# alipay/PainlessInferenceAcceleration

Hardware: NVIDIA H100
Metric: accepted tokens/sec @ Llama-2-7B 64-draft/8-branch; mean accepted len/step (higher is better)
Workload: dtype bf16

## Files before the change

include/pia_b200.h:

```cpp
#ifndef PIA_B200_H_
#define PIA_B200_H_

#include <stdint.h>

#ifdef __cplusplus
extern "C" {
#endif

#define PIA_ABI_VERSION 2

typedef enum {
  PIA_OK = 0,
  PIA_ERR_INVALID = -1,
  PIA_ERR_INDEX = -2,
  PIA_ERR_CAPACITY = -3,
  PIA_ERR_CUDA = -4,
  PIA_ERR_UNSUPPORTED = -5
} pia_status;

const char *pia_last_error(void);
int pia_abi_version(void);
unsigned long long pia_launch_count(void);

typedef struct pia_trie pia_trie_t;
// ... 70 lines not shown
  const int32_t *d_pad_len;
  int64_t kv_slot_stride;
  int32_t kv_first_slot;
} pia_slots_t;

typedef struct pia_attn_plan pia_attn_plan_t;

typedef struct {
  int32_t n_q_heads, n_kv_heads, head_dim;
  int32_t max_seq;
  int32_t max_nodes;
  int32_t n_layers;
  int32_t kv_split_max;
  int32_t n_slots;
} pia_attn_config_t;

int pia_attn_plan_create(const pia_attn_config_t *cfg, void *d_k_cache, void *d_v_cache, pia_attn_plan_t **out);
int pia_attn_plan_destroy(pia_attn_plan_t *p);
int pia_attn_plan_set_debug(pia_attn_plan_t *p, void *d_timestamps);
int pia_attn_plan_grid(const pia_attn_plan_t *p, int *n_split, int *n_groups);

int pia_tree_attn_fwd(pia_attn_plan_t *p, int layer, const void *d_q, const uint64_t *d_mask, const pia_slots_t *slots,
                      float scale_mul, void *d_out, void *stream);

int pia_tree_attn_fused_fwd(pia_attn_plan_t *p, int layer, const void *d_qkv, const void *d_cos, const void *d_sin,
                            int max_pos, const uint64_t *d_mask, const pia_slots_t *slots, float scale_mul, void *d_out,
                            void *stream);

typedef struct pia_gemm_plan pia_gemm_plan_t;
int pia_gemm_plan_create(const void *d_w, int N, int K, const void *d_x, int x_rows, int split_k, int w_tiled,
                         pia_gemm_plan_t **out);
int pia_gemm_plan_create_grouped(const void *d_w, int groups, int N, int K, const void *d_x, int x_rows,
                                 pia_gemm_plan_t **out);
int pia_gemm_plan_destroy(pia_gemm_plan_t *g);
int pia_gemm_plan_splits(const pia_gemm_plan_t *g);
int pia_gemm_plan_set_pdl(pia_gemm_plan_t *g, int on);
int pia_gemm_plan_set_silu(pia_gemm_plan_t *g, int on);
int pia_gemm_run(pia_gemm_plan_t *g, int rows, void *d_out, void *stream);

int pia_rmsnorm(const void *d_x, const void *d_residual_in, const void *d_weight, float eps, int rows, int hidden,
                void *d_residual_out, void *d_y, void *stream);
int pia_rmsnorm_partials(const float *d_x_parts, int n_parts, int64_t part_stride, const void *d_residual_in,
                         const void *d_weight, float eps, int rows, int hidden, void *d_residual_out, void *d_y,
                         void *stream);
int pia_rope_kv_append(const void *d_qkv, const uint64_t *d_mask, int mask_words, const pia_slots_t *slots,
                       int n_q_heads, int n_kv_heads, int head_dim, const void *d_cos, const void *d_sin, int max_pos,
// ... 47 lines not shown
```

painlessinferenceacceleration_b200/_lib.py:

```python
import ctypes as C
import os

from .build import SO

_lib = None

i32p = C.POINTER(C.c_int32)
u64p = C.POINTER(C.c_uint64)
vp = C.c_void_p

PIA_OK, PIA_ERR_INVALID, PIA_ERR_INDEX, PIA_ERR_CAPACITY, PIA_ERR_CUDA, PIA_ERR_UNSUPPORTED = 0, -1, -2, -3, -4, -5
MODE = {'input': 0, 'output': 1, 'mix': 2}
GET_HIER, GET_ONE = 0, 1
GET_TAIL = 1
GET_FIRST_ONLY = 2


class TrieConfig(C.Structure):
    _fields_ = [('vocab_capacity', C.c_int32), ('node_capacity', C.c_int64), ('edge_capacity', C.c_int64),
                ('n_input_slots', C.c_int32), ('max_node', C.c_int32), ('max_output_node', C.c_int32),
                ('max_put_tokens', C.c_int32), ('frontier_capacity', C.c_int32), ('max_resident_queries', C.c_int32)]


class TrieStats(C.Structure):
# ... 28 lines not shown
    'pia_trie_set_limits': (C.c_int, [vp, C.c_int, C.c_int]),
    'pia_trie_put': (C.c_int, [vp, vp, C.c_int, vp, C.c_int, C.c_int, C.c_int, C.c_int, vp]),
    'pia_trie_tree_put': (C.c_int, [vp, C.c_int, vp, C.c_int, C.c_int, C.c_int, vp]),
    'pia_trie_stream_put': (C.c_int, [vp, vp, C.c_int, vp, C.c_int, C.c_int, vp, C.c_int, vp]),
    'pia_trie_get': (C.c_int, [vp, vp, vp, C.c_int, C.c_int, C.c_int, vp, C.c_int, C.c_int, C.c_int, C.c_int, C.c_int,
                               C.c_int, C.c_int, C.c_int, C.c_int, vp, vp, vp, vp, vp, vp, vp, vp]),
    'pia_trie_tree_squeeze': (C.c_int, [vp, C.c_int, vp]),
    'pia_trie_tree_reset_input_freq': (C.c_int, [vp, C.c_int, C.c_int, vp]),
    'pia_trie_reset_input_freqs': (C.c_int, [vp, C.c_int, vp]),
    'pia_trie_squeeze_branch_counts': (C.c_int, [vp, vp]),
    'pia_trie_fresh': (C.c_int, [vp, vp]),
    'pia_trie_stats': (C.c_int, [vp, C.POINTER(TrieStats), vp]),
    'pia_trie_copy_error_flags': (C.c_int, [vp, vp, vp]),
    'pia_trie_tree_counters': (C.c_int, [vp, C.c_int, C.POINTER(C.c_int64), C.POINTER(C.c_int64), vp]),
    'pia_trie_compact': (C.c_int, [vp, C.POINTER(C.c_int64), C.POINTER(C.c_int64), vp]),
    'pia_trie_export_sizes': (C.c_int, [vp, C.POINTER(C.c_int64), C.POINTER(C.c_int64), vp]),
    'pia_trie_export': (C.c_int, [vp, vp, C.c_int64, vp, C.c_int64, vp, vp, vp, vp]),
    'pia_trie_import': (C.c_int, [vp, vp, C.c_int64, vp, C.c_int64, vp, vp, vp, vp]),
    'pia_attn_plan_create': (C.c_int, [C.POINTER(AttnConfig), vp, vp, C.POINTER(vp)]),
    'pia_attn_plan_destroy': (C.c_int, [vp]),
    'pia_attn_plan_set_debug': (C.c_int, [vp, vp]),
    'pia_attn_plan_grid': (C.c_int, [vp, C.POINTER(C.c_int), C.POINTER(C.c_int)]),
    'pia_tree_attn_fwd': (C.c_int, [vp, C.c_int, vp, vp, C.POINTER(Slots), C.c_float, vp, vp]),
    'pia_tree_attn_fused_fwd': (C.c_int, [vp, C.c_int, vp, vp, vp, C.c_int, vp, C.POINTER(Slots), C.c_float, vp, vp]),
    'pia_rmsnorm': (C.c_int, [vp, vp, vp, C.c_float, C.c_int, C.c_int, vp, vp, vp]),
    'pia_rmsnorm_partials': (C.c_int, [vp, C.c_int, C.c_int64, vp, vp, C.c_float, C.c_int, C.c_int, vp, vp, vp]),
    'pia_gemm_plan_create': (C.c_int, [vp, C.c_int, C.c_int, vp, C.c_int, C.c_int, C.c_int, C.POINTER(vp)]),
    'pia_gemm_plan_create_grouped': (C.c_int, [vp, C.c_int, C.c_int, C.c_int, vp, C.c_int, C.POINTER(vp)]),
    'pia_gemm_plan_destroy': (C.c_int, [vp]),
    'pia_gemm_plan_splits': (C.c_int, [vp]),
    'pia_gemm_plan_set_pdl': (C.c_int, [vp, C.c_int]),
    'pia_gemm_plan_set_silu': (C.c_int, [vp, C.c_int]),
    'pia_gemm_run': (C.c_int, [vp, C.c_int, vp, vp]),
    'pia_rope_kv_append': (C.c_int, [vp, vp, C.c_int, C.POINTER(Slots), C.c_int, C.c_int, C.c_int, vp, vp,
                                     C.c_int, vp, vp, vp, C.c_int, vp]),
    'pia_silu_mul': (C.c_int, [vp, C.c_int, C.c_int, vp, vp]),
    'pia_embed_gather': (C.c_int, [vp, vp, vp, C.c_int, C.c_int, vp, vp]),
    'pia_moe_combine': (C.c_int, [vp, vp, C.c_int, C.c_int, C.c_int, C.c_int, vp, vp]),
    'pia_moe_router': (C.c_int, [vp, vp, C.c_int, C.c_int, C.c_int, C.c_int, vp, vp]),
    'pia_l2_prefetch': (C.c_int, [vp, C.c_int64, C.c_int64, C.c_int64, C.c_float, vp]),
    'pia_accept': (C.c_int, [C.POINTER(AcceptConfig), vp, vp, vp, C.c_int, C.c_int, C.c_int, vp, vp, vp, C.c_int, vp,
                             vp, vp, vp, vp, vp, vp, vp, vp]),
    'pia_accept_workspace_bytes': (C.c_int64, [C.POINTER(AcceptConfig)]),
    'pia_kv_compact': (C.c_int, [vp, vp, C.c_int, C.c_int, C.c_int, C.c_int, C.c_int, C.c_int64, vp, C.c_int, vp, vp,
                                 vp]),
    'pia_flood_update_draft_table': (C.c_int, [vp, C.c_int, vp, vp, C.c_int64, C.c_int, C.c_int, C.c_int, vp]),
# ... 36 lines not shown
```

painlessinferenceacceleration_b200/common/ops.py:

```python
import ctypes as C

import torch

from .. import _lib as L


def _s():
    return torch.cuda.current_stream().cuda_stream


def _p(t):
    return t.data_ptr() if t is not None else None


def rmsnorm(x, residual_in, weight, eps, residual_out, y):
    rows, hidden = x.shape
    L.check(L.load().pia_rmsnorm(_p(x), _p(residual_in), _p(weight), float(eps), rows, hidden, _p(residual_out),
                                 _p(y), _s()))


def rmsnorm_partials(parts, residual_in, weight, eps, residual_out, y):
    n_parts, prow, hidden = parts.shape
    rows = y.shape[0]
    L.check(L.load().pia_rmsnorm_partials(_p(parts), n_parts, prow * hidden, _p(residual_in), _p(weight), float(eps),
# ... 124 lines not shown
    L.check(L.load().pia_l2_prefetch(t.data_ptr() + offset_bytes, int(n_ranges), int(stride_bytes), int(range_bytes),
                                     float(gbytes_per_s), _s()))


def embed_gather(table, ids, n, out):
    rows, hidden = out.shape
    L.check(L.load().pia_embed_gather(_p(table), _p(ids), _p(n), rows, hidden, _p(out), _s()))


class AttnPlan(object):

    def __init__(self, k_cache, v_cache, n_q_heads, n_kv_heads, head_dim, max_nodes, kv_split_max=0):
        n_slots = k_cache.shape[0] if k_cache.dim() == 5 else 1
        n_layers, hkv, max_seq, hd = k_cache.shape[-4:]
        assert hkv == n_kv_heads and hd == head_dim and k_cache.is_contiguous() and v_cache.is_contiguous()
        self.cfg = L.AttnConfig(n_q_heads, n_kv_heads, head_dim, max_seq, max_nodes, n_layers, kv_split_max, n_slots)
        self.slot_stride = n_layers * hkv * max_seq * hd
        self.h = L.vp()
        self.lib = L.load()
        with torch.cuda.device(k_cache.device):
            L.check(self.lib.pia_attn_plan_create(C.byref(self.cfg), _p(k_cache), _p(v_cache), C.byref(self.h)))
        self._keep = (k_cache, v_cache)

    def forward(self, layer, q, mask, slots, out, scale_mul=1.0):
        assert q.shape[0] >= slots.rows and mask.shape[0] >= slots.rows and out.shape[0] >= slots.rows
        L.check(self.lib.pia_tree_attn_fwd(self.h, layer, _p(q), _p(mask), slots.ref(), float(scale_mul), _p(out), _s()))

    def forward_fused(self, layer, qkv, mask, slots, cos, sin, out, scale_mul=1.0):
        assert qkv.shape[0] >= slots.rows and mask.shape[0] >= slots.rows and out.shape[0] >= slots.rows
        L.check(self.lib.pia_tree_attn_fused_fwd(self.h, layer, _p(qkv), _p(cos), _p(sin), cos.shape[0], _p(mask),
                                                 slots.ref(), float(scale_mul), _p(out), _s()))

    def close(self):
        if self.h:
            self.lib.pia_attn_plan_destroy(self.h)
            self.h = None

    def __del__(self):
        try:
            self.close()
        except Exception:
            pass


class Accept(object):

    def __init__(self, vocab, max_nodes, repetition_penalty, eos_ids, max_length, device, bound_walk=False):
        eos = [int(e) for e in (eos_ids or []) if e is not None][:8]
        arr = (C.c_int32 * 8)(*(eos + [-1] * (8 - len(eos))))
# ... 27 lines not shown
```

painlessinferenceacceleration_b200/csrc/tree_attn.cu:

```cuda
#include <cuda.h>
#include <cuda_bf16.h>

#include <stdlib.h>

#include <new>

#include "common.cuh"

namespace pia {
namespace attn {

constexpr int BN = 128;
constexpr int HD = 128;
constexpr int NSTAGE = 2;
constexpr int NTHREADS = 288;
constexpr int PRODUCER_WARP = 8;
constexpr int SUB = 128 * 128;
constexpr int TILE_BYTES = 2 * SUB;
constexpr int SMEM_Q = 0, SMEM_K = TILE_BYTES, SMEM_V = SMEM_K + NSTAGE * TILE_BYTES;
constexpr int SMEM_BAR = SMEM_V + NSTAGE * TILE_BYTES;
constexpr int MRG_ACC = 0;
constexpr int MRG_ML = 112 * 1024;
constexpr int MRG_DED_ACC = SMEM_BAR + 256, MRG_DED_ACC_BYTES = (64 + 8) * 128 * 4,
               MRG_DED_ML = MRG_DED_ACC + MRG_DED_ACC_BYTES;
constexpr int SMEM_TOTAL = MRG_DED_ML + 1024 + 1024;
constexpr int MAX_SPLIT = 8;
// ... 93 lines not shown
  for (int j = 0; j < 8; ++j) {
    const float x = __bfloat162float(a.h[j]);
    const float r = lower ? -__bfloat162float(b.h[j]) : __bfloat162float(b.h[j]);
    o.h[j] = __float2bfloat16_rn(bfr(x * __bfloat162float(c.h[j])) + bfr(r * __bfloat162float(s.h[j])));
  }
  return o.u;
}

struct Params {
  const __nv_bfloat16 *q;
  const unsigned long long *mask;
  pia_slots_t sl;
  int slot_planes;
  int plane0;
  int layer, n_q_heads, n_kv_heads, np, mask_words, heads_per_cta, max_seq, n_split, tiles_per_cta;
  float scale_log2;
  int fused;
  const __nv_bfloat16 *qkv;
  const __nv_bfloat16 *cos_t, *sin_t;
  int max_pos;
  __nv_bfloat16 *kc_layer, *vc_layer;
  __nv_bfloat16 *out;
  unsigned long long *dbg;
};

__device__ __forceinline__ unsigned long long gtime() {
  unsigned long long t;
  asm volatile("mov.u64 %0, %%globaltimer;" : "=l"(t));
  return t;
}
#define DBG(ev) do { if (p.dbg) p.dbg[((size_t)blockIdx.y * gridDim.x + blockIdx.x) * 16 + (ev)] = gtime(); } while (0)

__global__ void __launch_bounds__(NTHREADS, 1)
k_tree_attn(const __grid_constant__ CUtensorMap map_k, const __grid_constant__ CUtensorMap map_v, Params p) {
  extern __shared__ uint8_t smem_raw[];
  const uint32_t base = (smem_u32(smem_raw) + 1023u) & ~1023u;
  uint8_t *sm = smem_raw + (base - smem_u32(smem_raw));
  const int tid = threadIdx.x, warp = tid >> 5, lane = tid & 31;

  const uint32_t bar0 = base + SMEM_BAR;
  const uint32_t bar_kv_full = bar0, bar_kv_empty = bar0 + 8 * NSTAGE, bar_v_full = bar0 + 16 * NSTAGE;

  pdl_launch_dependents();
  if (tid == 0) {
    asm volatile("prefetch.tensormap [%0];" ::"l"(reinterpret_cast<unsigned long long>(&map_k)) : "memory");
    asm volatile("prefetch.tensormap [%0];" ::"l"(reinterpret_cast<unsigned long long>(&map_v)) : "memory");
  }
  const int split = blockIdx.x, group = blockIdx.y;
  const int slot = blockIdx.z;
  const int n = p.sl.d_n[slot], P = p.sl.d_prefix_len[slot];
  const int pad_len = p.sl.d_pad_len ? p.sl.d_pad_len[slot] : 0;
  if (n <= 0) return;
  const long long row0 = (long long)slot * p.sl.rows_per_slot;
  const int L = P + n;
  const int hq0 = group * p.heads_per_cta;
  const int hkv = hq0 / (p.n_q_heads / p.n_kv_heads);
  const bool fused = p.fused != 0;
  const int Tp = (P + BN - 1) / BN;
  const int tiles_total = fused ? Tp + 1 : (L + BN - 1) / BN;
  const int rows_used = p.heads_per_cta * p.np;
  const int n_wg = rows_used / 64;
  const bool ded = (rows_used + MAX_SPLIT) * HD * 4 <= MRG_DED_ACC_BYTES;
  int ns = (tiles_total + p.tiles_per_cta - 1) / p.tiles_per_cta;
  if (ns > p.n_split) ns = p.n_split;
  if (ns < 1) ns = 1;
  if (split >= ns) {
    if (ns > 1) { cluster_sync_all(); cluster_sync_all(); }
    return;
  }
  const int tps = (tiles_total + ns - 1) / ns;
  const int t0 = split * tps;
  int t1 = t0 + tps;
  if (t1 > tiles_total) t1 = tiles_total;
  const int ntile = t1 - t0;
  const bool has_draft = fused && ntile > 0 && t1 == tiles_total;
  auto tile_of = [&](int i) -> int { return has_draft ? (i == 0 ? Tp : t0 + i - 1) : t0 + i; };
  if (ns > 1 && ded) cluster_arrive();
  auto barrier_a = [&]() { if (ded) cluster_wait(); else cluster_sync_all(); };
  const int mrg_acc = ded ? MRG_DED_ACC : MRG_ACC, mrg_ml = ded ? MRG_DED_ML : MRG_ML;
  const int mrg_stride = ded ? 64 + MAX_SPLIT : 128 + MAX_SPLIT;
  if (tid == 0) DBG(0);

  if (tid == 0) {
    for (int s = 0; s < NSTAGE; ++s) {
      mbar_init(bar_kv_full + 8 * s, 1); mbar_init(bar_v_full + 8 * s, 1);
      mbar_init(bar_kv_empty + 8 * s, 4 * n_wg);
    }
    asm volatile("fence.mbarrier_init.release.cluster;" ::: "memory");
  }
  __syncwarp();
  __syncthreads();
  if (tid == 0) DBG(1);

  if (warp == PRODUCER_WARP) {
    if (lane == 0 && ntile > 0) {
      const int plane = p.plane0 + slot * p.slot_planes + p.layer * p.n_kv_heads + hkv;
      int p_safe = P;
      if (p.slot_planes == 0) for (int b2 = 0; b2 < p.sl.batch; ++b2) p_safe = min(p_safe, p.sl.d_prefix_len[b2]);
      bool waited = false;
      for (int i = 0; i < ntile; ++i) {
        const int s = i % NSTAGE, ph = (i / NSTAGE) & 1;
        if (has_draft && i == 0) {
          mbar_arrive(bar_kv_full);
          mbar_arrive(bar_v_full);
          continue;
        }
        const int key0 = tile_of(i) * BN;
        if (!fused && !waited && key0 + BN > p_safe) { pdl_wait(); waited = true; }
        mbar_wait(bar_kv_empty + 8 * s, ph ^ 1);
        const uint32_t kd = base + SMEM_K + s * TILE_BYTES, vd = base + SMEM_V + s * TILE_BYTES;
        mbar_expect_tx(bar_kv_full + 8 * s, TILE_BYTES);
        tma_load_3d(kd, &map_k, bar_kv_full + 8 * s, 0, key0, plane);
        tma_load_3d(kd + SUB, &map_k, bar_kv_full + 8 * s, 64, key0, plane);
        mbar_expect_tx(bar_v_full + 8 * s, TILE_BYTES);
        tma_load_3d(vd, &map_v, bar_v_full + 8 * s, 0, key0, plane);
        tma_load_3d(vd + SUB, &map_v, bar_v_full + 8 * s, 64, key0, plane);
        if (i == 0) DBG(2);
      }
    }
    __syncwarp();
    if (ns > 1) { barrier_a(); cluster_sync_all(); }
  } else {
    pdl_wait();
    {
      const int srow = tid & 127, half = tid >> 7;
      const int hs = srow / p.np, node = srow % p.np;
      if (srow < rows_used) {
        if (!fused) {
          uint4 qv[8];
          const bool have = hs < p.heads_per_cta && node < n;
          const uint4 *src = reinterpret_cast<const uint4 *>(p.q + ((row0 + node) * p.n_q_heads + hq0 + hs) * HD) + half * 8;
#pragma unroll
          for (int ch = 0; ch < 8; ++ch) qv[ch] = have ? src[ch] : make_uint4(0, 0, 0, 0);
#pragma unroll
          for (int ch = 0; ch < 8; ++ch)
            *reinterpret_cast<uint4 *>(sm + SMEM_Q + half * SUB + srow * 128 + ((ch ^ (srow & 7)) << 4)) = qv[ch];
        } else {
          unsigned long long mr0 = 0ull, mr1 = 0ull;
          if (node < n) {
            mr0 = p.mask[(row0 + node) * p.mask_words];
            if (p.mask_words > 1) mr1 = p.mask[(row0 + node) * p.mask_words + 1];
          }
          int pos = (P > pad_len ? P - pad_len : 0) + __popcll(mr0) + __popcll(mr1) - 1;
          pos = pos < 0 ? 0 : (pos >= p.max_pos ? p.max_pos - 1 : pos);
// ... 201 lines not shown
        __syncwarp();
        if (lane == 0) mbar_arrive(bar_kv_empty + 8 * s);
      }
      if (tid == 0) DBG(8);
#pragma unroll
      for (int h = 0; h < 2; ++h) {
        l_run[h] += __shfl_xor_sync(FULL, l_run[h], 1);
        l_run[h] += __shfl_xor_sync(FULL, l_run[h], 2);
      }
      if (tid == 0) DBG(9);
      if (ns == 1) {
#pragma unroll
        for (int h = 0; h < 2; ++h) {
          if (live[h]) {
            const float inv = l_run[h] > 0.f ? 1.f / l_run[h] : 0.f;
            uint32_t *dst = reinterpret_cast<uint32_t *>(p.out + ((row0 + node[h]) * p.n_q_heads + hq0 + hs[h]) * HD);
#pragma unroll
            for (int nb = 0; nb < 16; ++nb) {
              __nv_bfloat162 b = __floats2bfloat162_rn(o[4 * nb + 2 * h] * inv, o[4 * nb + 2 * h + 1] * inv);
              dst[4 * nb + (lane & 3)] = *reinterpret_cast<uint32_t *>(&b);
            }
          }
        }
      } else {
        barrier_a();
        if (tid == 0) DBG(14);
        const int RS = (rows_used + ns - 1) / ns;
#pragma unroll
        for (int h = 0; h < 2; ++h) {
          if (live[h]) {
            const int owner = rw[h] / RS, rl = rw[h] % RS;
            const uint32_t dst = map_to_cta(base + mrg_acc + (uint32_t)((((lane & 3) >> 1) * mrg_stride + split * RS + rl) * 16 + (lane & 1) * 8), owner);
#pragma unroll
            for (int nb = 0; nb < 16; ++nb)
              st_cluster_f2(dst + (uint32_t)(2 * nb * mrg_stride) * 16, o[4 * nb + 2 * h], o[4 * nb + 2 * h + 1]);
            if ((lane & 3) == 0) st_cluster_f2(map_to_cta(base + mrg_ml + (uint32_t)(split * RS + rl) * 8, owner), m_run[h], l_run[h]);
          }
        }
        __syncwarp();
        if (tid == 0) DBG(15);
        cluster_sync_all();
      }
      if (tid == 0) DBG(10);
    } else {
      if (ns > 1) { barrier_a(); cluster_sync_all(); }
    }
  }
  if (ns > 1) {
    const int RS = (rows_used + ns - 1) / ns;
    const float4 *macc = reinterpret_cast<const float4 *>(sm + mrg_acc);
    const float2 *mml = reinterpret_cast<const float2 *>(sm + mrg_ml);
    const int items = RS * (HD / 4);
    const bool pow2 = (RS & (RS - 1)) == 0 && (p.np & (p.np - 1)) == 0;
    const int rs_sh = 31 - __clz(RS), np_sh = 31 - __clz(p.np);
    for (int it = tid; it < items; it += NTHREADS) {
      const int rl = pow2 ? (it & (RS - 1)) : it % RS, c4 = pow2 ? (it >> rs_sh) : it / RS;
      const int r = split * RS + rl;
      if (r >= rows_used) continue;
      const int rh = pow2 ? (r >> np_sh) : r / p.np, rn = pow2 ? (r & (p.np - 1)) : r % p.np;
      if (rn >= n) continue;
      float2 ml[MAX_SPLIT];
      float4 a4[MAX_SPLIT];
#pragma unroll
      for (int i = 0; i < MAX_SPLIT; ++i) {
        if (i < ns) { ml[i] = mml[i * RS + rl]; a4[i] = macc[c4 * mrg_stride + i * RS + rl]; }
        else { ml[i] = make_float2(-INFINITY, 0.f); a4[i] = make_float4(0.f, 0.f, 0.f, 0.f); }
      }
      float M = -INFINITY;
#pragma unroll
      for (int i = 0; i < MAX_SPLIT; ++i) M = fmaxf(M, ml[i].x);
      float den = 0.f;
      float4 o4 = make_float4(0.f, 0.f, 0.f, 0.f);
#pragma unroll
      for (int i = 0; i < MAX_SPLIT; ++i) {
        const float w = ml[i].x == -INFINITY ? 0.f : ex2(ml[i].x - M);
        den += ml[i].y * w;
        o4.x += a4[i].x * w; o4.y += a4[i].y * w; o4.z += a4[i].z * w; o4.w += a4[i].w * w;
      }
      const float inv = den > 0.f ? 1.f / den : 0.f;
      __nv_bfloat162 b0 = __floats2bfloat162_rn(o4.x * inv, o4.y * inv), b1 = __floats2bfloat162_rn(o4.z * inv, o4.w * inv);
      reinterpret_cast<uint2 *>(p.out + ((row0 + rn) * p.n_q_heads + hq0 + rh) * HD)[c4] =
          make_uint2(*reinterpret_cast<uint32_t *>(&b0), *reinterpret_cast<uint32_t *>(&b1));
    }
  }
  if (tid == 0) DBG(12);
}

}
}

using namespace pia;
using namespace pia::attn;

struct pia_attn_plan {
  pia_attn_config_t cfg;
  CUtensorMap map_k, map_v;
  int heads_per_cta, n_groups, n_split, mask_words, tiles_per_cta;
  unsigned long long *dbg;
  __nv_bfloat16 *k_base, *v_base;
};

typedef CUresult (*EncodeTiledFn)(CUtensorMap *, CUtensorMapDataType, cuuint32_t, void *, const cuuint64_t *,
                                  const cuuint64_t *, const cuuint32_t *, const cuuint32_t *, CUtensorMapInterleave,
                                  CUtensorMapSwizzle, CUtensorMapL2promotion, CUtensorMapFloatOOBfill);

static int encode_kv_map(CUtensorMap *m, void *base, const pia_attn_config_t &c) {
  static EncodeTiledFn fn = nullptr;
  if (!fn) {
    cudaDriverEntryPointQueryResult qres;
    void *ptr = nullptr;
    PIA_CUDA_CHECK(cudaGetDriverEntryPoint("cuTensorMapEncodeTiled", &ptr, cudaEnableDefault, &qres));
    PIA_REQUIRE(ptr && qres == cudaDriverEntryPointSuccess, "cuTensorMapEncodeTiled not available in this driver");
    fn = (EncodeTiledFn)ptr;
  }
  cuuint64_t dims[3] = {(cuuint64_t)c.head_dim, (cuuint64_t)c.max_seq,
                        (cuuint64_t)(c.n_slots > 0 ? c.n_slots : 1) * c.n_layers * c.n_kv_heads};
  cuuint64_t strides[2] = {(cuuint64_t)c.head_dim * 2, (cuuint64_t)c.max_seq * c.head_dim * 2};
  cuuint32_t box[3] = {64, (cuuint32_t)BN, 1};
  cuuint32_t estr[3] = {1, 1, 1};
  CUresult r = fn(m, CU_TENSOR_MAP_DATA_TYPE_BFLOAT16, 3, base, dims, strides, box, estr, CU_TENSOR_MAP_INTERLEAVE_NONE,
                  CU_TENSOR_MAP_SWIZZLE_128B, CU_TENSOR_MAP_L2_PROMOTION_L2_256B, CU_TENSOR_MAP_FLOAT_OOB_FILL_NONE);
  if (r != CUDA_SUCCESS) { set_error("cuTensorMapEncodeTiled failed with CUresult %d", (int)r); return PIA_ERR_CUDA; }
// ... 14 lines not shown
  const int G = cfg->n_q_heads / cfg->n_kv_heads;
  p->heads_per_cta = (cfg->max_nodes == 64 && G % 2 == 0) ? 2 : 1;
  p->n_groups = cfg->n_q_heads / p->heads_per_cta;
  p->mask_words = cfg->max_nodes / 64;
  int n_sm = 132, dev = 0;
  cudaGetDevice(&dev);
  cudaDeviceGetAttribute(&n_sm, cudaDevAttrMultiProcessorCount, dev);
  const int max_tiles = (cfg->max_seq + BN - 1) / BN;
  int ns = cfg->kv_split_max > 0 ? cfg->kv_split_max : n_sm / p->n_groups;
  if (ns > max_tiles) ns = max_tiles;
  if (ns < 1) ns = 1;
  if (ns > MAX_SPLIT) ns = MAX_SPLIT;
  p->n_split = ns;
  p->tiles_per_cta = 1;
  if (const char *e = getenv("PIA_ATTN_TILES_PER_CTA")) { int v = atoi(e); if (v >= 1 && v <= 64) p->tiles_per_cta = v; }
  int rc = encode_kv_map(&p->map_k, d_k_cache, *cfg);
  if (rc == PIA_OK) rc = encode_kv_map(&p->map_v, d_v_cache, *cfg);
  if (rc == PIA_OK) {
    cudaError_t e = cudaFuncSetAttribute(k_tree_attn, cudaFuncAttributeMaxDynamicSharedMemorySize, SMEM_TOTAL);
    if (e != cudaSuccess) { set_error("cudaFuncSetAttribute: %s", cudaGetErrorString(e)); rc = PIA_ERR_CUDA; }
  }
  p->dbg = nullptr;
  p->k_base = (__nv_bfloat16 *)d_k_cache; p->v_base = (__nv_bfloat16 *)d_v_cache;
  if (rc != PIA_OK) { delete p; return rc; }
  *out = p;
  return PIA_OK;
}

extern "C" int pia_attn_plan_set_debug(pia_attn_plan_t *p, void *d_timestamps) {
  PIA_REQUIRE(p, "null plan");
  p->dbg = (unsigned long long *)d_timestamps;
  return PIA_OK;
}
extern "C" int pia_attn_plan_grid(const pia_attn_plan_t *p, int *n_split, int *n_groups) {
  PIA_REQUIRE(p && n_split && n_groups, "null argument");
  *n_split = p->n_split; *n_groups = p->n_groups;
  return PIA_OK;
}

extern "C" int pia_attn_plan_destroy(pia_attn_plan_t *p) {
  if (p) delete p;
  return PIA_OK;
}

static int attn_launch(pia_attn_plan_t *p, int layer, const void *d_q, const void *d_qkv, const void *d_cos,
                       const void *d_sin, int max_pos, const uint64_t *d_mask, const pia_slots_t *slots, float scale_mul,
                       void *d_out, void *stream) {
  const bool fused = d_qkv != nullptr;
  PIA_REQUIRE(p && (d_q || d_qkv) && d_mask && slots && slots->d_n && slots->d_prefix_len && d_out, "null argument");
  PIA_REQUIRE(layer >= 0 && layer < p->cfg.n_layers, "layer %d outside [0,%d)", layer, p->cfg.n_layers);
  PIA_REQUIRE(slots->batch >= 1 && slots->batch <= 65535 && slots->rows_per_slot >= 1 &&
                  slots->rows_per_slot <= p->cfg.max_nodes, "bad slot table");
  const long long cache_elems = (long long)p->cfg.n_layers * p->cfg.n_kv_heads * p->cfg.max_seq * p->cfg.head_dim;
  const int plan_slots = p->cfg.n_slots > 0 ? p->cfg.n_slots : 1;
  PIA_REQUIRE(slots->kv_first_slot >= 0 && slots->kv_first_slot < plan_slots, "kv_first_slot outside the plan's caches");
  PIA_REQUIRE(slots->kv_slot_stride == 0 || (slots->kv_slot_stride == cache_elems &&
                                              slots->kv_first_slot + slots->batch <= plan_slots),
              "kv_slot_stride must be 0 or one whole cache, and the plan must span `batch` caches");
  PIA_REQUIRE(!fused || slots->batch == 1 || slots->kv_slot_stride != 0,
              "the fused RoPE / KV-append attention needs one cache per slot");
  PIA_REQUIRE(!fused || (d_cos && d_sin && max_pos > 0), "fused mode needs the RoPE tables");
  Params a;
  a.q = (const __nv_bfloat16 *)d_q;
  a.mask = (const unsigned long long *)d_mask;
  a.sl = *slots;
  a.slot_planes = slots->kv_slot_stride ? p->cfg.n_layers * p->cfg.n_kv_heads : 0;
  a.plane0 = slots->kv_first_slot * p->cfg.n_layers * p->cfg.n_kv_heads;
  a.layer = layer; a.n_q_heads = p->cfg.n_q_heads; a.n_kv_heads = p->cfg.n_kv_heads; a.np = p->cfg.max_nodes;
  a.mask_words = p->mask_words; a.heads_per_cta = p->heads_per_cta; a.max_seq = p->cfg.max_seq;
  int ns = p->n_split / slots->batch;
  if (ns < 1) ns = 1;
  a.n_split = ns; a.tiles_per_cta = p->tiles_per_cta;
  a.out = (__nv_bfloat16 *)d_out; a.dbg = p->dbg;
  a.fused = fused ? 1 : 0;
  a.qkv = (const __nv_bfloat16 *)d_qkv; a.cos_t = (const __nv_bfloat16 *)d_cos; a.sin_t = (const __nv_bfloat16 *)d_sin;
  a.max_pos = max_pos;
  const long long layer_off = ((long long)slots->kv_first_slot * p->cfg.n_layers + layer) * p->cfg.n_kv_heads *
                              (long long)p->cfg.max_seq * p->cfg.head_dim;
  a.kc_layer = p->k_base + layer_off; a.vc_layer = p->v_base + layer_off;
  a.scale_log2 = scale_mul * 1.4426950408889634f / sqrtf((float)HD);
  cudaStream_t s = (cudaStream_t)stream;
  PIA_CUDA_CHECK(launch_kernel_cluster(k_tree_attn, dim3(ns, p->n_groups, slots->batch), dim3(NTHREADS), SMEM_TOTAL, s,
                                       (unsigned)ns, p->map_k, p->map_v, a));
  count_launch();
  return PIA_OK;
}

extern "C" int pia_tree_attn_fwd(pia_attn_plan_t *p, int layer, const void *d_q, const uint64_t *d_mask,
                                 const pia_slots_t *slots, float scale_mul, void *d_out, void *stream) {
  PIA_REQUIRE(d_q, "null q");
  return attn_launch(p, layer, d_q, nullptr, nullptr, nullptr, 0, d_mask, slots, scale_mul, d_out, stream);
}

extern "C" int pia_tree_attn_fused_fwd(pia_attn_plan_t *p, int layer, const void *d_qkv, const void *d_cos,
                                       const void *d_sin, int max_pos, const uint64_t *d_mask, const pia_slots_t *slots,
                                       float scale_mul, void *d_out, void *stream) {
  PIA_REQUIRE(d_qkv, "null qkv");
  return attn_launch(p, layer, nullptr, d_qkv, d_cos, d_sin, max_pos, d_mask, slots, scale_mul, d_out, stream);
}
```

painlessinferenceacceleration_b200/models/llama/modeling_llama.py:

```python
import glob
import json
import os

import torch
from torch import nn

from ...common import ops
from ...common.pretrained_model import LookaheadPreTrainedModel


class LlamaRMSNorm(nn.Module):
    def __init__(self, hidden_size, eps=1e-6, device=None, dtype=None):
        super().__init__()
        self.weight = nn.Parameter(torch.ones(hidden_size, device=device, dtype=dtype))
        self.variance_epsilon = eps


class LlamaAttention(nn.Module):
    def __init__(self, cfg, device, dtype):
        super().__init__()
        hd = cfg.hidden_size // cfg.num_attention_heads
        kv = getattr(cfg, 'num_key_value_heads', None) or cfg.num_attention_heads
        kw = dict(bias=False, device=device, dtype=dtype)
        self.q_proj = nn.Linear(cfg.hidden_size, cfg.num_attention_heads * hd, **kw)
# ... 174 lines not shown
        if 'qkv' in want:
            plans['qkv'] = self._mk_gemm(layer.self_attn.qkv_weight, b.y)
        sk = int(os.environ.get('PIA_GEMM_SPLIT', '-4'))
        if 'qkv2' in want:
            plans['qkv'] = self._mk_gemm(layer.self_attn.qkv_weight, b.y, split_k=-2)
        if 'o' in want:
            plans['o'] = self._mk_gemm(layer.self_attn.o_proj.weight.data, b.attn, split_k=sk)
        if 'down' in want and layer.mlp.down_proj.weight.shape[1] % 64 == 0 and layer.mlp.down_proj.weight.shape[1] >= 64 * abs(sk):
            plans['down'] = self._mk_gemm(layer.mlp.down_proj.weight.data, b.act, split_k=sk)
        for name in os.environ.get('PIA_GEMM_NOPDL', '').split(','):
            if name in plans:
                plans[name].set_pdl(False)
        return plans

    def _mk_gemm(self, w, x, split_k=1):
        if w.shape[0] % 128 == 0:
            cache = self.__dict__.setdefault('_tiled_weights', {})
            key = (w.data_ptr(), tuple(w.shape))
            if key not in cache:
                cache[key] = ops.tile_weight(w)
            return ops.Gemm(cache[key], x, split_k=split_k, tiled=True)
        return ops.Gemm(w.contiguous(), x, split_k=split_k)

    def _prefetch_cfg(self, rt):
        cfg = getattr(rt, 'prefetch_cfg', None)
        if cfg is None:
            import os
            spec = os.environ.get('PIA_PREFETCH', '0')
            v = [float(t) for t in spec.split(',')] if spec not in ('', '0') else []
            cfg = False
            if v and torch.cuda.is_available():
                v = (v + [0.0] * 4)[:4]
                cfg = dict(o=v[0], gate_up=v[1], down=v[2], rate=v[3], side=torch.cuda.Stream(device=self.device))
            rt.prefetch_cfg = cfg
        return cfg

    @staticmethod
    def _prefetch(pf, jobs):
        main = torch.cuda.current_stream()
        pf['side'].wait_stream(main)
        with torch.cuda.stream(pf['side']):
            for (t, frac, tile_bytes) in jobs:
                if frac <= 0:
                    continue
                total = t.numel() * t.element_size()
                if tile_bytes:
                    rb = max(16384, int(tile_bytes * min(frac, 1.0)) // 16384 * 16384)
                    ops.l2_prefetch(t, n_ranges=total // tile_bytes, stride_bytes=tile_bytes, range_bytes=min(rb, tile_bytes),
                                    gbytes_per_s=pf['rate'])
                else:
                    ops.l2_prefetch(t, range_bytes=int(total * min(frac, 1.0)) // 16 * 16, gbytes_per_s=pf['rate'])
        pf['dirty'] = True

    def _mlp(self, rt, layer, y, plans=None, pf=None):
        m = layer.mlp
        if plans:
# ... 5 lines not shown
                    plans['gate_up'].run(64, out=b.gu)
                else:
                    torch.mm(y, m.gate_up_weight.t(), out=b.gu)
                if pf:
                    self._prefetch(pf, [(m.down_proj.weight, pf['down'], 0)])
                ops.silu_mul(b.gu, b.act)
            if 'down' in plans:
                o = plans['down'].run(64)
                return (o, None) if plans['down'].splits == 1 else (None, o)
            return torch.mm(b.act, m.down_proj.weight.t()), None
        gu = torch.mm(y, m.gate_up_weight.t())
        act = torch.empty((gu.shape[0], gu.shape[1] // 2), dtype=gu.dtype, device=gu.device)
        ops.silu_mul(gu, act)
        return torch.mm(act, m.down_proj.weight.t()), None

    def _verify_layers(self, rt, bufs=None, last_only=False):
        self.fuse()
        b = bufs if bufs is not None else rt.decode_bufs
        g = rt.g
        eps = self.config.rms_norm_eps
        ops.embed_gather(self.model.embed_tokens.weight, b.ids, b.n_total, b.h)
        plans = self._gemm_plans(rt) if b is rt.decode_bufs else False
        pf = self._prefetch_cfg(rt) if plans else False
        fused_attn = b is rt.decode_bufs and os.environ.get('PIA_ATTN_FUSED', '0') != '0' and \
            (b.slots.batch == 1 or b.slots.kv_slot_stride != 0)
        x, parts, resid_in = b.h, None, None

        def norm(w):
            if parts is not None:
                ops.rmsnorm_partials(parts, resid_in, w, eps, b.resid, b.y)
            else:
                ops.rmsnorm(x, resid_in, w, eps, b.resid, b.y)

        for li, layer in enumerate(self.model.layers):
            lp = plans['layers'][li] if plans else None
            norm(layer.input_layernorm.weight)
            a = layer.self_attn
            if lp and 'qkv' in lp:
                lp['qkv'].run(64, out=b.qkv)
            else:
                torch.mm(b.y, a.qkv_weight.t(), out=b.qkv)
            if pf and lp and 'gate_up' in lp:
                gw = lp['gate_up'].weight
                self._prefetch(pf, [(a.o_proj.weight, pf['o'], 0),
                                    (gw, pf['gate_up'], gw.shape[1] * gw.shape[2] * gw.shape[3] * 2 if gw.dim() == 4 else 0)])
            if fused_attn:
                rt.plan.forward_fused(li, b.qkv, b.mask, b.slots, rt.rope_cos, rt.rope_sin, b.attn)
            else:
                ops.rope_kv_append(b.qkv, b.mask, b.slots, g['n_q_heads'], g['n_kv_heads'], g['head_dim'], rt.rope_cos,
                                   rt.rope_sin, b.q, rt.k_layer(li, b.kv_slot), rt.v_layer(li, b.kv_slot), rt.max_seq)
                rt.plan.forward(li, b.q, b.mask, b.slots, b.attn)
            if lp and 'o' in lp:
                o = lp['o'].run(64)
                x, parts, resid_in = (o, None, b.resid) if lp['o'].splits == 1 else (None, o, b.resid)
            else:
                x, parts, resid_in = torch.mm(b.attn, a.o_proj.weight.t()), None, b.resid
            norm(layer.post_attention_layernorm.weight)
            x, parts = self._mlp(rt, layer, b.y, lp, pf)
        if pf and pf.pop('dirty', False):
            torch.cuda.current_stream().wait_stream(pf['side'])
        if last_only:
            return
        norm(self.model.norm.weight)
        if b.logits is not None:
            if plans:
                plans['lm_head'].run(64, out=b.logits)
            else:
                torch.mm(b.y, self.lm_head.weight.t(), out=b.logits)


class LlamaPreTrainedModel(LookaheadPreTrainedModel):
    pass
```

Measured before the change: 528.6.

## Add global-memory split merge and in-kernel L2 prefetch to tree attention

Adds an alternative split-KV merge that writes partial results to a global workspace and lets the last-arriving CTA (via an atomic counter) combine them. This path is chosen automatically when the required clusters exceed occupancy, avoiding cluster launch limits and cluster barriers. It also lets the attention kernel issue bulk L2 prefetches of the o_proj weight while it runs, replacing the side-stream o_proj prefetch. The cost is extra global traffic and workspace memory, plus a changed PIA_PREFETCH format.

Result: faster. 546.1 (median of 6 runs) (+3.3%).

```diff
diff --git a/include/pia_b200.h b/include/pia_b200.h
--- a/include/pia_b200.h
+++ b/include/pia_b200.h
@@ -116,6 +116,9 @@
 
 int pia_tree_attn_fwd(pia_attn_plan_t *p, int layer, const void *d_q, const uint64_t *d_mask, const pia_slots_t *slots,
                       float scale_mul, void *d_out, void *stream);
+int pia_tree_attn_prefetch_fwd(pia_attn_plan_t *p, int layer, const void *d_q, const uint64_t *d_mask,
+                               const pia_slots_t *slots, float scale_mul, void *d_out, const void *d_l2, int64_t l2_bytes,
+                               void *stream);
 
 int pia_tree_attn_fused_fwd(pia_attn_plan_t *p, int layer, const void *d_qkv, const void *d_cos, const void *d_sin,
                             int max_pos, const uint64_t *d_mask, const pia_slots_t *slots, float scale_mul, void *d_out,
diff --git a/painlessinferenceacceleration_b200/_lib.py b/painlessinferenceacceleration_b200/_lib.py
--- a/painlessinferenceacceleration_b200/_lib.py
+++ b/painlessinferenceacceleration_b200/_lib.py
@@ -74,6 +74,7 @@
     'pia_attn_plan_set_debug': (C.c_int, [vp, vp]),
     'pia_attn_plan_grid': (C.c_int, [vp, C.POINTER(C.c_int), C.POINTER(C.c_int)]),
     'pia_tree_attn_fwd': (C.c_int, [vp, C.c_int, vp, vp, C.POINTER(Slots), C.c_float, vp, vp]),
+    'pia_tree_attn_prefetch_fwd': (C.c_int, [vp, C.c_int, vp, vp, C.POINTER(Slots), C.c_float, vp, vp, C.c_int64, vp]),
     'pia_tree_attn_fused_fwd': (C.c_int, [vp, C.c_int, vp, vp, vp, C.c_int, vp, C.POINTER(Slots), C.c_float, vp, vp]),
     'pia_rmsnorm': (C.c_int, [vp, vp, vp, C.c_float, C.c_int, C.c_int, vp, vp, vp]),
     'pia_rmsnorm_partials': (C.c_int, [vp, C.c_int, C.c_int64, vp, vp, C.c_float, C.c_int, C.c_int, vp, vp, vp]),
diff --git a/painlessinferenceacceleration_b200/common/ops.py b/painlessinferenceacceleration_b200/common/ops.py
--- a/painlessinferenceacceleration_b200/common/ops.py
+++ b/painlessinferenceacceleration_b200/common/ops.py
@@ -170,9 +170,16 @@
             L.check(self.lib.pia_attn_plan_create(C.byref(self.cfg), _p(k_cache), _p(v_cache), C.byref(self.h)))
         self._keep = (k_cache, v_cache)
 
-    def forward(self, layer, q, mask, slots, out, scale_mul=1.0):
+    def forward(self, layer, q, mask, slots, out, scale_mul=1.0, l2_prefetch=None, l2_prefetch_bytes=None):
         assert q.shape[0] >= slots.rows and mask.shape[0] >= slots.rows and out.shape[0] >= slots.rows
-        L.check(self.lib.pia_tree_attn_fwd(self.h, layer, _p(q), _p(mask), slots.ref(), float(scale_mul), _p(out), _s()))
+        if l2_prefetch is None:
+            L.check(self.lib.pia_tree_attn_fwd(self.h, layer, _p(q), _p(mask), slots.ref(), float(scale_mul), _p(out),
+                                               _s()))
+            return
+        total = l2_prefetch.numel() * l2_prefetch.element_size()
+        nb = total if l2_prefetch_bytes is None else min(int(l2_prefetch_bytes), total)
+        L.check(self.lib.pia_tree_attn_prefetch_fwd(self.h, layer, _p(q), _p(mask), slots.ref(), float(scale_mul),
+                                                    _p(out), _p(l2_prefetch), nb // 16 * 16, _s()))
 
     def forward_fused(self, layer, qkv, mask, slots, cos, sin, out, scale_mul=1.0):
         assert qkv.shape[0] >= slots.rows and mask.shape[0] >= slots.rows and out.shape[0] >= slots.rows
diff --git a/painlessinferenceacceleration_b200/csrc/tree_attn.cu b/painlessinferenceacceleration_b200/csrc/tree_attn.cu
--- a/painlessinferenceacceleration_b200/csrc/tree_attn.cu
+++ b/painlessinferenceacceleration_b200/csrc/tree_attn.cu
@@ -2,6 +2,7 @@
 #include <cuda_bf16.h>
 
 #include <stdlib.h>
+#include <string.h>
 
 #include <new>
 
@@ -141,7 +142,73 @@
   __nv_bfloat16 *kc_layer, *vc_layer;
   __nv_bfloat16 *out;
   unsigned long long *dbg;
+  const char *l2_base;
+  long long l2_bytes;
+  int gmerge;
+  float4 *gm_acc;
+  float2 *gm_ml;
+  int *gm_count;
 };
+
+template <int NSM>
+__device__ __forceinline__ uint2 combine4(const float2 (&ml)[NSM], const float4 (&a4)[NSM]) {
+  float M = -INFINITY;
+#pragma unroll
+  for (int i = 0; i < NSM; ++i) M = fmaxf(M, ml[i].x);
+  float den = 0.f;
+  float4 o4 = make_float4(0.f, 0.f, 0.f, 0.f);
+#pragma unroll
+  for (int i = 0; i < NSM; ++i) {
+    const float w = ml[i].x == -INFINITY ? 0.f : ex2(ml[i].x - M);
+    den += ml[i].y * w;
+    o4.x += a4[i].x * w; o4.y += a4[i].y * w; o4.z += a4[i].z * w; o4.w += a4[i].w * w;
+  }
+  const float inv = den > 0.f ? 1.f / den : 0.f;
+  __nv_bfloat162 b0 = __floats2bfloat162_rn(o4.x * inv, o4.y * inv), b1 = __floats2bfloat162_rn(o4.z * inv, o4.w * inv);
+  return make_uint2(*reinterpret_cast<uint32_t *>(&b0), *reinterpret_cast<uint32_t *>(&b1));
+}
+
+constexpr int L2_CHUNK = 16384;
+
+__device__ __forceinline__ void l2_prefetch_share(const Params &p) {
+  if (p.l2_bytes <= 0) return;
+  const long long n_cta = (long long)gridDim.x * gridDim.y * gridDim.z;
+  const long long cta = ((long long)blockIdx.z * gridDim.y + blockIdx.y) * gridDim.x + blockIdx.x;
+  for (long long off = cta * L2_CHUNK; off < p.l2_bytes; off += n_cta * L2_CHUNK) {
+    const long long left = p.l2_bytes - off;
+    const uint32_t sz = (uint32_t)(left < L2_CHUNK ? left : L2_CHUNK);
+    asm volatile("cp.async.bulk.prefetch.L2.global [%0], %1;" ::"l"(p.l2_base + off), "r"(sz) : "memory");
+  }
+}
+
+template <int NSM, int PER>
+__device__ __forceinline__ void gm_combine(const Params &p, size_t g0, int rows_used, int n, int ns, long long row0, int hq0,
+                                           int tid) {
+  const int items = rows_used * (HD / 4);
+  for (int it0 = tid; it0 < items; it0 += PER * NTHREADS) {
+    float2 ml[PER][NSM];
+    float4 a4[PER][NSM];
+    bool ok[PER];
+#pragma unroll
+    for (int k = 0; k < PER; ++k) {
+      const int it = it0 + k * NTHREADS, r = it >> 5, c4 = it & 31;
+      ok[k] = it < items && r % p.np < n;
+#pragma unroll
+      for (int i = 0; i < NSM; ++i) {
+        if (ok[k] && i < ns) {
+          ml[k][i] = __ldcg(p.gm_ml + g0 + i * 128 + r);
+          a4[k][i] = __ldcg(p.gm_acc + (g0 + i * 128 + r) * (HD / 4) + c4);
+        } else { ml[k][i] = make_float2(-INFINITY, 0.f); a4[k][i] = make_float4(0.f, 0.f, 0.f, 0.f); }
+      }
+    }
+#pragma unroll
+    for (int k = 0; k < PER; ++k) {
+      const int it = it0 + k * NTHREADS, r = it >> 5, c4 = it & 31;
+      if (ok[k])
+        reinterpret_cast<uint2 *>(p.out + ((row0 + r % p.np) * p.n_q_heads + hq0 + r / p.np) * HD)[c4] = combine4(ml[k], a4[k]);
+    }
+  }
+}
 
 __device__ __forceinline__ unsigned long long gtime() {
   unsigned long long t;
@@ -183,8 +250,9 @@
   int ns = (tiles_total + p.tiles_per_cta - 1) / p.tiles_per_cta;
   if (ns > p.n_split) ns = p.n_split;
   if (ns < 1) ns = 1;
+  const bool gm = p.gmerge != 0;
   if (split >= ns) {
-    if (ns > 1) { cluster_sync_all(); cluster_sync_all(); }
+    if (ns > 1 && !gm) { cluster_sync_all(); cluster_sync_all(); }
     return;
   }
   const int tps = (tiles_total + ns - 1) / ns;
@@ -194,7 +262,7 @@
   const int ntile = t1 - t0;
   const bool has_draft = fused && ntile > 0 && t1 == tiles_total;
   auto tile_of = [&](int i) -> int { return has_draft ? (i == 0 ? Tp : t0 + i - 1) : t0 + i; };
-  if (ns > 1 && ded) cluster_arrive();
+  if (ns > 1 && ded && !gm) cluster_arrive();
   auto barrier_a = [&]() { if (ded) cluster_wait(); else cluster_sync_all(); };
   const int mrg_acc = ded ? MRG_DED_ACC : MRG_ACC, mrg_ml = ded ? MRG_DED_ML : MRG_ML;
   const int mrg_stride = ded ? 64 + MAX_SPLIT : 128 + MAX_SPLIT;
@@ -237,8 +305,9 @@
         if (i == 0) DBG(2);
       }
     }
+    if (lane == 0) l2_prefetch_share(p);
     __syncwarp();
-    if (ns > 1) { barrier_a(); cluster_sync_all(); }
+    if (ns > 1 && !gm) { barrier_a(); cluster_sync_all(); }
   } else {
     pdl_wait();
     {
@@ -486,6 +555,17 @@
             }
           }
         }
+      } else if (gm) {
+        const size_t g0 = ((size_t)blockIdx.z * gridDim.y + group) * p.n_split * 128 + (size_t)split * 128;
+#pragma unroll
+        for (int h = 0; h < 2; ++h) {
+          if (live[h]) {
+            float2 *dst = reinterpret_cast<float2 *>(p.gm_acc + (g0 + rw[h]) * (HD / 4)) + (lane & 3);
+#pragma unroll
+            for (int nb = 0; nb < 16; ++nb) dst[4 * nb] = make_float2(o[4 * nb + 2 * h], o[4 * nb + 2 * h + 1]);
+            if ((lane & 3) == 0) p.gm_ml[g0 + rw[h]] = make_float2(m_run[h], l_run[h]);
+          }
+        }
       } else {
         barrier_a();
         if (tid == 0) DBG(14);
@@ -507,10 +587,27 @@
       }
       if (tid == 0) DBG(10);
     } else {
-      if (ns > 1) { barrier_a(); cluster_sync_all(); }
+      if (ns > 1 && !gm) { barrier_a(); cluster_sync_all(); }
     }
   }
-  if (ns > 1) {
+  if (ns > 1 && gm) {
+    __syncthreads();
+    if (tid == 0) DBG(14);
+    int *last = reinterpret_cast<int *>(sm + SMEM_BAR + 128);
+    int *cnt = p.gm_count + (size_t)blockIdx.z * gridDim.y + group;
+    if (tid == 0) {
+      int old;
+      asm volatile("atom.acq_rel.gpu.global.add.s32 %0, [%1], 1;" : "=r"(old) : "l"(cnt) : "memory");
+      const int is_last = old == ns - 1;
+      if (is_last) asm volatile("st.relaxed.gpu.global.s32 [%0], 0;" ::"l"(cnt) : "memory");
+      *last = is_last;
+    }
+    __syncthreads();
+    if (!*last) return;
+    if (tid == 0) DBG(15);
+    const size_t g0 = ((size_t)blockIdx.z * gridDim.y + group) * p.n_split * 128;
+    gm_combine<MAX_SPLIT, 2>(p, g0, rows_used, n, ns, row0, hq0, tid);
+  } else if (ns > 1) {
     const int RS = (rows_used + ns - 1) / ns;
     const float4 *macc = reinterpret_cast<const float4 *>(sm + mrg_acc);
     const float2 *mml = reinterpret_cast<const float2 *>(sm + mrg_ml);
@@ -530,21 +627,7 @@
         if (i < ns) { ml[i] = mml[i * RS + rl]; a4[i] = macc[c4 * mrg_stride + i * RS + rl]; }
         else { ml[i] = make_float2(-INFINITY, 0.f); a4[i] = make_float4(0.f, 0.f, 0.f, 0.f); }
       }
-      float M = -INFINITY;
-#pragma unroll
-      for (int i = 0; i < MAX_SPLIT; ++i) M = fmaxf(M, ml[i].x);
-      float den = 0.f;
-      float4 o4 = make_float4(0.f, 0.f, 0.f, 0.f);
-#pragma unroll
-      for (int i = 0; i < MAX_SPLIT; ++i) {
-        const float w = ml[i].x == -INFINITY ? 0.f : ex2(ml[i].x - M);
-        den += ml[i].y * w;
-        o4.x += a4[i].x * w; o4.y += a4[i].y * w; o4.z += a4[i].z * w; o4.w += a4[i].w * w;
-      }
-      const float inv = den > 0.f ? 1.f / den : 0.f;
-      __nv_bfloat162 b0 = __floats2bfloat162_rn(o4.x * inv, o4.y * inv), b1 = __floats2bfloat162_rn(o4.z * inv, o4.w * inv);
-      reinterpret_cast<uint2 *>(p.out + ((row0 + rn) * p.n_q_heads + hq0 + rh) * HD)[c4] =
-          make_uint2(*reinterpret_cast<uint32_t *>(&b0), *reinterpret_cast<uint32_t *>(&b1));
+      reinterpret_cast<uint2 *>(p.out + ((row0 + rn) * p.n_q_heads + hq0 + rh) * HD)[c4] = combine4(ml, a4);
     }
   }
   if (tid == 0) DBG(12);
@@ -562,6 +645,11 @@
   int heads_per_cta, n_groups, n_split, mask_words, tiles_per_cta;
   unsigned long long *dbg;
   __nv_bfloat16 *k_base, *v_base;
+  int max_clusters[MAX_SPLIT + 1];
+  int merge_mode;
+  float4 *gm_acc;
+  float2 *gm_ml;
+  int *gm_count;
 };
 
 typedef CUresult (*EncodeTiledFn)(CUtensorMap *, CUtensorMapDataType, cuuint32_t, void *, const cuuint64_t *,
@@ -622,7 +710,33 @@
   }
   p->dbg = nullptr;
   p->k_base = (__nv_bfloat16 *)d_k_cache; p->v_base = (__nv_bfloat16 *)d_v_cache;
-  if (rc != PIA_OK) { delete p; return rc; }
+  p->merge_mode = 0;
+  if (const char *e = getenv("PIA_ATTN_MERGE")) p->merge_mode = !strcmp(e, "cluster") ? 1 : !strcmp(e, "global") ? 2 : 0;
+  for (int c = 0; c <= MAX_SPLIT; ++c) p->max_clusters[c] = 1 << 30;
+  for (int c = 2; rc == PIA_OK && c <= ns; ++c) {
+    cudaLaunchConfig_t lc = {};
+    lc.gridDim = dim3(c, p->n_groups, 1); lc.blockDim = dim3(NTHREADS); lc.dynamicSmemBytes = SMEM_TOTAL;
+    cudaLaunchAttribute at;
+    at.id = cudaLaunchAttributeClusterDimension;
+    at.val.clusterDim.x = c; at.val.clusterDim.y = 1; at.val.clusterDim.z = 1;
+    lc.attrs = &at; lc.numAttrs = 1;
+    int nc = 0;
+    if (cudaOccupancyMaxActiveClusters(&nc, k_tree_attn, &lc) == cudaSuccess && nc > 0) p->max_clusters[c] = nc;
+    else cudaGetLastError();
+  }
+  p->gm_acc = nullptr; p->gm_ml = nullptr; p->gm_count = nullptr;
+  if (rc == PIA_OK && ns > 1) {
+    const size_t rows = (size_t)p->n_groups * ns * 128, groups = (size_t)p->n_groups * ns;
+    if (cudaMalloc(&p->gm_acc, rows * HD * sizeof(float)) != cudaSuccess ||
+        cudaMalloc(&p->gm_ml, rows * sizeof(float2)) != cudaSuccess ||
+        cudaMalloc(&p->gm_count, groups * sizeof(int)) != cudaSuccess ||
+        cudaMemset(p->gm_count, 0, groups * sizeof(int)) != cudaSuccess) {
+      cudaGetLastError();
+      set_error("out of device memory for the attention merge workspace");
+      rc = PIA_ERR_CUDA;
+    }
+  }
+  if (rc != PIA_OK) { pia_attn_plan_destroy(p); return rc; }
   *out = p;
   return PIA_OK;
 }
@@ -639,15 +753,20 @@
 }
 
 extern "C" int pia_attn_plan_destroy(pia_attn_plan_t *p) {
-  if (p) delete p;
+  if (p) {
+    cudaFree(p->gm_acc); cudaFree(p->gm_ml); cudaFree(p->gm_count);
+    delete p;
+  }
   return PIA_OK;
 }
 
 static int attn_launch(pia_attn_plan_t *p, int layer, const void *d_q, const void *d_qkv, const void *d_cos,
                        const void *d_sin, int max_pos, const uint64_t *d_mask, const pia_slots_t *slots, float scale_mul,
-                       void *d_out, void *stream) {
+                       void *d_out, void *stream, const void *d_l2 = nullptr, int64_t l2_bytes = 0) {
   const bool fused = d_qkv != nullptr;
   PIA_REQUIRE(p && (d_q || d_qkv) && d_mask && slots && slots->d_n && slots->d_prefix_len && d_out, "null argument");
+  PIA_REQUIRE(l2_bytes >= 0 && (l2_bytes == 0 || (d_l2 && l2_bytes % 16 == 0 && ((uintptr_t)d_l2 & 15) == 0)),
+              "L2 prefetch range must be 16-byte aligned and a multiple of 16 bytes");
   PIA_REQUIRE(layer >= 0 && layer < p->cfg.n_layers, "layer %d outside [0,%d)", layer, p->cfg.n_layers);
   PIA_REQUIRE(slots->batch >= 1 && slots->batch <= 65535 && slots->rows_per_slot >= 1 &&
                   slots->rows_per_slot <= p->cfg.max_nodes, "bad slot table");
@@ -672,6 +791,10 @@
   if (ns < 1) ns = 1;
   a.n_split = ns; a.tiles_per_cta = p->tiles_per_cta;
   a.out = (__nv_bfloat16 *)d_out; a.dbg = p->dbg;
+  a.l2_base = (const char *)d_l2; a.l2_bytes = l2_bytes;
+  const int clusters = p->n_groups * slots->batch;
+  a.gmerge = ns > 1 && (p->merge_mode == 2 || (p->merge_mode == 0 && clusters > p->max_clusters[ns])) ? 1 : 0;
+  a.gm_acc = p->gm_acc; a.gm_ml = p->gm_ml; a.gm_count = p->gm_count;
   a.fused = fused ? 1 : 0;
   a.qkv = (const __nv_bfloat16 *)d_qkv; a.cos_t = (const __nv_bfloat16 *)d_cos; a.sin_t = (const __nv_bfloat16 *)d_sin;
   a.max_pos = max_pos;
@@ -681,7 +804,7 @@
   a.scale_log2 = scale_mul * 1.4426950408889634f / sqrtf((float)HD);
   cudaStream_t s = (cudaStream_t)stream;
   PIA_CUDA_CHECK(launch_kernel_cluster(k_tree_attn, dim3(ns, p->n_groups, slots->batch), dim3(NTHREADS), SMEM_TOTAL, s,
-                                       (unsigned)ns, p->map_k, p->map_v, a));
+                                       a.gmerge ? 1u : (unsigned)ns, p->map_k, p->map_v, a));
   count_launch();
   return PIA_OK;
 }
@@ -690,6 +813,14 @@
                                  const pia_slots_t *slots, float scale_mul, void *d_out, void *stream) {
   PIA_REQUIRE(d_q, "null q");
   return attn_launch(p, layer, d_q, nullptr, nullptr, nullptr, 0, d_mask, slots, scale_mul, d_out, stream);
+}
+
+extern "C" int pia_tree_attn_prefetch_fwd(pia_attn_plan_t *p, int layer, const void *d_q, const uint64_t *d_mask,
+                                          const pia_slots_t *slots, float scale_mul, void *d_out, const void *d_l2,
+                                          int64_t l2_bytes, void *stream) {
+  PIA_REQUIRE(d_q, "null q");
+  return attn_launch(p, layer, d_q, nullptr, nullptr, nullptr, 0, d_mask, slots, scale_mul, d_out, stream, d_l2,
+                     l2_bytes);
 }
 
 extern "C" int pia_tree_attn_fused_fwd(pia_attn_plan_t *p, int layer, const void *d_qkv, const void *d_cos,
diff --git a/painlessinferenceacceleration_b200/models/llama/modeling_llama.py b/painlessinferenceacceleration_b200/models/llama/modeling_llama.py
--- a/painlessinferenceacceleration_b200/models/llama/modeling_llama.py
+++ b/painlessinferenceacceleration_b200/models/llama/modeling_llama.py
@@ -220,16 +220,24 @@
             return ops.Gemm(cache[key], x, split_k=split_k, tiled=True)
         return ops.Gemm(w.contiguous(), x, split_k=split_k)
 
+    def _attn_l2_bytes(self, rt):
+        nb = getattr(rt, 'attn_l2_bytes', None)
+        if nb is None:
+            frac = min(max(float(os.environ.get('PIA_ATTN_L2_PREFETCH', '0.5')), 0.0), 1.0)
+            w = self.model.layers[0].self_attn.o_proj.weight
+            nb = int(w.numel() * w.element_size() * frac) // 16 * 16
+            rt.attn_l2_bytes = nb
+        return nb
+
     def _prefetch_cfg(self, rt):
         cfg = getattr(rt, 'prefetch_cfg', None)
         if cfg is None:
-            import os
             spec = os.environ.get('PIA_PREFETCH', '0')
             v = [float(t) for t in spec.split(',')] if spec not in ('', '0') else []
             cfg = False
             if v and torch.cuda.is_available():
-                v = (v + [0.0] * 4)[:4]
-                cfg = dict(o=v[0], gate_up=v[1], down=v[2], rate=v[3], side=torch.cuda.Stream(device=self.device))
+                v = (v + [0.0] * 3)[:3]
+                cfg = dict(gate_up=v[0], down=v[1], rate=v[2], side=torch.cuda.Stream(device=self.device))
             rt.prefetch_cfg = cfg
         return cfg
 
@@ -281,6 +289,7 @@
         ops.embed_gather(self.model.embed_tokens.weight, b.ids, b.n_total, b.h)
         plans = self._gemm_plans(rt) if b is rt.decode_bufs else False
         pf = self._prefetch_cfg(rt) if plans else False
+        l2_bytes = self._attn_l2_bytes(rt) if plans else 0
         fused_attn = b is rt.decode_bufs and os.environ.get('PIA_ATTN_FUSED', '0') != '0' and \
             (b.slots.batch == 1 or b.slots.kv_slot_stride != 0)
         x, parts, resid_in = b.h, None, None
@@ -301,14 +310,16 @@
                 torch.mm(b.y, a.qkv_weight.t(), out=b.qkv)
             if pf and lp and 'gate_up' in lp:
                 gw = lp['gate_up'].weight
-                self._prefetch(pf, [(a.o_proj.weight, pf['o'], 0),
-                                    (gw, pf['gate_up'], gw.shape[1] * gw.shape[2] * gw.shape[3] * 2 if gw.dim() == 4 else 0)])
+                self._prefetch(pf, [(gw, pf['gate_up'], gw.shape[1] * gw.shape[2] * gw.shape[3] * 2 if gw.dim() == 4 else 0)])
             if fused_attn:
                 rt.plan.forward_fused(li, b.qkv, b.mask, b.slots, rt.rope_cos, rt.rope_sin, b.attn)
             else:
                 ops.rope_kv_append(b.qkv, b.mask, b.slots, g['n_q_heads'], g['n_kv_heads'], g['head_dim'], rt.rope_cos,
                                    rt.rope_sin, b.q, rt.k_layer(li, b.kv_slot), rt.v_layer(li, b.kv_slot), rt.max_seq)
-                rt.plan.forward(li, b.q, b.mask, b.slots, b.attn)
+                if plans and not (lp and 'o' in lp) and l2_bytes:
+                    rt.plan.forward(li, b.q, b.mask, b.slots, b.attn, l2_prefetch=a.o_proj.weight, l2_prefetch_bytes=l2_bytes)
+                else:
+                    rt.plan.forward(li, b.q, b.mask, b.slots, b.attn)
             if lp and 'o' in lp:
                 o = lp['o'].run(64)
                 x, parts, resid_in = (o, None, b.resid) if lp['o'].splits == 1 else (None, o, b.resid)
```
